# autonomousvision/LaRa

Hardware: AMD Instinct MI355X
Metric: novel-view frames/sec @512x512 (4-view in, 2DGS fwd+bwd) (higher is better)
Workload: dtype f32 raster + bf16-MFMA/f32-accumulate encoder (+ bf16-autocast coarse decoder MLP, as the reference's bf16-mixed)

## Files before the change

include/lara_finedec.h:

```cpp
#ifndef LARA_FINEDEC_H
#define LARA_FINEDEC_H

#include <stdint.h>

#ifdef __cplusplus
extern "C" {
#endif

int lara_fine_decoder_forward(int32_t n, const float *xn, const float *pf, const float *Wqk, const float *W1ov,
                              const float *b1, const float *W2, const float *b2, float *sh, void *stream);

int lara_fine_decoder_backward(int32_t n, const float *xn, const float *pf, const float *Wqk, const float *W1ov,
                               const float *b1, const float *W2, const float *b2, const float *d_sh, float *d_xn,
                               float *d_pf, float *U, float *HID, float *DH, float *DT, void *stream);

int32_t lara_fine_wgrad_floats(void);
int64_t lara_fine_wgrad_workspace_bytes(int32_t n);
int lara_fine_decoder_wgrad(int32_t n, const float *xn, const float *U, const float *HID, const float *DH, const float *DT,
                            const float *d_sh, float *out, void *workspace, void *stream);

int32_t lara_fine_ln_blocks(int32_t n);
int lara_fine_ln_forward(int32_t n, const float *x, const float *gamma, const float *beta, float eps, float *xn,
                         float *stats, void *stream);
int lara_fine_ln_backward(int32_t n, const float *x, const float *gamma, const float *stats, const float *d_xn,
                          float *d_x, float *partials, void *stream);

#ifdef __cplusplus
}
#endif
#endif
```

lara_amd/csrc/finedec.hip:

```cpp
#include "common.h"
#include "../../include/lara_finedec.h"

namespace {

constexpr int FD = 80, NH = 8, CD = 8, NV = 4, HID = 64, SH = 12, TQ = NH * CD;

typedef float f32x16 __attribute__((ext_vector_type(16)));

__device__ __forceinline__ int crow(const int tile, const int r, const int hf) { return tile * 32 + (r >> 2) * 8 + hf * 4 + (r & 3); }
__device__ __forceinline__ f32x16 mfma2(const float a, const float b, const f32x16 c) {
    return __builtin_amdgcn_mfma_f32_32x32x2f32(a, b, c, 0, 0, 0);
}
#define FD_FENCE(i, every) do { if (((i) % (every)) == (every) - 1) asm volatile("" ::: "memory"); } while (0)

__device__ __forceinline__ f32x16 zero16() {
    f32x16 z;
#pragma unroll
    for (int i = 0; i < 16; i++) z[i] = 0.f;
    return z;
}

constexpr int L_WQKT = 0;
constexpr int L_W1T = L_WQKT + FD * TQ;
constexpr int L_W2T = L_W1T + TQ * HID;
// ... 26 lines not shown
    for (int k = 0; k < 10; k++) { const float4 v = x4[k]; xh[4 * k] = v.x; xh[4 * k + 1] = v.y; xh[4 * k + 2] = v.z; xh[4 * k + 3] = v.w; }
}

__device__ __forceinline__ void folded_queries(const float *sw, const float xh[40], const int col, const int hf, f32x16 t[2]) {
    t[0] = zero16(); t[1] = zero16();
#pragma unroll
    for (int s = 0; s < 40; s++) {
        const float *w = sw + L_WQKT + (hf * 40 + s) * TQ + col;
        t[0] = mfma2(w[0], xh[s], t[0]);
        t[1] = mfma2(w[32], xh[s], t[1]);
        FD_FENCE(s, 4);
    }
}

__device__ __forceinline__ void load_pf_half(const float *pf_g, const int64_t n, const int64_t pt, const int hf, float pf[NV][4]) {
#pragma unroll
    for (int j = 0; j < NV; j++)
#pragma unroll
        for (int c = 0; c < 4; c++) pf[j][c] = pf_g[(int64_t)(j * CD + hf * 4 + c) * n + pt];
}

__device__ __forceinline__ float other_half(const float x) { return __shfl_xor(x, 32, 64); }

__device__ __forceinline__ void attention_weights(const f32x16 t[2], const float pf[NV][4], float p[NH][NV]) {
#pragma unroll
    for (int h = 0; h < NH; h++) {
        float sc[NV], m = -1e30f;
#pragma unroll
        for (int j = 0; j < NV; j++) {
            float a = 0.f;
#pragma unroll
            for (int c = 0; c < 4; c++) a += t[h >> 2][(h & 3) * 4 + c] * pf[j][c];
            a += other_half(a);
            sc[j] = a;
            m = fmaxf(m, a);
        }
        float z = 0.f;
#pragma unroll
        for (int j = 0; j < NV; j++) { p[h][j] = __expf(sc[j] - m); z += p[h][j]; }
        const float rz = 1.0f / z;
#pragma unroll
        for (int j = 0; j < NV; j++) p[h][j] *= rz;
    }
}

__device__ __forceinline__ void attend(const float p[NH][NV], const float pf[NV][4], f32x16 u[2]) {
#pragma unroll
    for (int h = 0; h < NH; h++)
#pragma unroll
        for (int c = 0; c < 4; c++)
            u[h >> 2][(h & 3) * 4 + c] = p[h][0] * pf[0][c] + p[h][1] * pf[1][c] + p[h][2] * pf[2][c] + p[h][3] * pf[3][c];
}

__device__ __forceinline__ void hidden_pre(const float *sw, const f32x16 u[2], const int col, const int hf, f32x16 hid[2]) {
    hid[0] = zero16(); hid[1] = zero16();
#pragma unroll
    for (int mt = 0; mt < 2; mt++)
#pragma unroll
        for (int r = 0; r < 16; r++) {
            const float *w = sw + L_W1T + crow(mt, r, hf) * HID + col;
            hid[0] = mfma2(w[0], u[mt][r], hid[0]);
            hid[1] = mfma2(w[32], u[mt][r], hid[1]);
            FD_FENCE(r, 4);
        }
#pragma unroll
    for (int mt = 0; mt < 2; mt++)
#pragma unroll
        for (int r = 0; r < 16; r++) hid[mt][r] += sw[L_B1 + crow(mt, r, hf)];
}

__global__ void __launch_bounds__(256) __attribute__((amdgpu_waves_per_eu(2, 2)))
fine_decoder_fwd_kernel(const int n, const float *__restrict__ xn_g, const float *__restrict__ pf_g,
                        const float *__restrict__ Wqk, const float *__restrict__ W1ov, const float *__restrict__ b1,
                        const float *__restrict__ W2, const float *__restrict__ b2, float *__restrict__ sh_g) {
    __shared__ __attribute__((aligned(16))) float sw[L_FWD_END];
    stage_weights(sw, Wqk, W1ov, b1, W2, b2, false);
    const int lane = threadIdx.x & 63, col = lane & 31, hf = lane >> 5, wave = threadIdx.x >> 6;
    for (int64_t base = (int64_t)blockIdx.x * 128; base < n; base += (int64_t)gridDim.x * 128) {
        const int64_t pt = base + wave * 32 + col;
        const bool live = pt < n;
        const int64_t ptc = live ? pt : (int64_t)n - 1;
        float xh[40];
        load_xn_half(xn_g, ptc, hf, xh);
        f32x16 tu[2];
        folded_queries(sw, xh, col, hf, tu);
        {
            float pf[NV][4], p[NH][NV];
            load_pf_half(pf_g, n, ptc, hf, pf);
            attention_weights(tu, pf, p);
            attend(p, pf, tu);
        }
        f32x16 hid[2];
        hidden_pre(sw, tu, col, hf, hid);
        f32x16 out = zero16();
#pragma unroll
        for (int mt = 0; mt < 2; mt++)
#pragma unroll
            for (int r = 0; r < 16; r++) {
                out = mfma2(sw[L_W2T + crow(mt, r, hf) * 32 + col], fmaxf(hid[mt][r], 0.f), out);
                FD_FENCE(r, 8);
            }
        if (live) {
            float4 *o4 = (float4 *)(sh_g + pt * SH);
            const float *bb = sw + L_B2;
            o4[hf] = make_float4(out[0] + bb[4 * hf], out[1] + bb[4 * hf + 1], out[2] + bb[4 * hf + 2], out[3] + bb[4 * hf + 3]);
            if (hf == 0) o4[2] = make_float4(out[4] + bb[8], out[5] + bb[9], out[6] + bb[10], out[7] + bb[11]);
        }
    }
}

__global__ void __launch_bounds__(256)
fine_decoder_bwd_kernel(const int n, const float *__restrict__ xn_g, const float *__restrict__ pf_g,
                        const float *__restrict__ Wqk, const float *__restrict__ W1ov, const float *__restrict__ b1,
                        const float *__restrict__ W2, const float *__restrict__ b2, const float *__restrict__ dsh_g,
                        float *__restrict__ dxn_g, float *__restrict__ dpf_g, float *__restrict__ U_g,
                        float *__restrict__ H_g, float *__restrict__ DH_g, float *__restrict__ DT_g) {
    extern __shared__ __attribute__((aligned(16))) float sw[];
    stage_weights(sw, Wqk, W1ov, b1, W2, b2, true);
    const int lane = threadIdx.x & 63, col = lane & 31, hf = lane >> 5, wave = threadIdx.x >> 6;
    auto store64 = [&](float *g, const int64_t pt, const f32x16 v[2]) {
#pragma unroll
        for (int mt = 0; mt < 2; mt++)
#pragma unroll
            for (int q = 0; q < 4; q++)
                *(float4 *)(g + pt * 64 + mt * 32 + q * 8 + hf * 4) = make_float4(v[mt][4 * q], v[mt][4 * q + 1], v[mt][4 * q + 2], v[mt][4 * q + 3]);
    };
    for (int64_t base = (int64_t)blockIdx.x * 128; base < n; base += (int64_t)gridDim.x * 128) {
        const int64_t pt = base + wave * 32 + col;
        const bool live = pt < n;
        const int64_t ptc = live ? pt : (int64_t)n - 1;
        f32x16 t[2], u[2];
        {
            float xh[40];
            load_xn_half(xn_g, ptc, hf, xh);
            folded_queries(sw, xh, col, hf, t);
        }
        float pf[NV][4], p[NH][NV];
        load_pf_half(pf_g, n, ptc, hf, pf);
        attention_weights(t, pf, p);
        attend(p, pf, u);
        if (live) store64(U_g, pt, u);
        asm volatile("" ::: "memory");
        f32x16 hid[2], dh[2];
        hidden_pre(sw, u, col, hf, hid);
        {
            float ds[8];
            const float4 *d4 = (const float4 *)(dsh_g + ptc * SH);
            if (hf == 0) {
                const float4 a = d4[0], b = d4[1];
                ds[0] = a.x; ds[1] = a.y; ds[2] = a.z; ds[3] = a.w; ds[4] = b.x; ds[5] = b.y; ds[6] = b.z; ds[7] = b.w;
            } else {
                const float4 c = d4[2];
                ds[0] = c.x; ds[1] = c.y; ds[2] = c.z; ds[3] = c.w; ds[4] = ds[5] = ds[6] = ds[7] = 0.f;
            }
            dh[0] = zero16(); dh[1] = zero16();
#pragma unroll
            for (int s_ = 0; s_ < 8; s_++) {
                const float *w = sw + L_W2P + (hf * 8 + s_) * HID + col;
                dh[0] = mfma2(w[0], ds[s_], dh[0]);
                dh[1] = mfma2(w[32], ds[s_], dh[1]);
                FD_FENCE(s_, 4);
// ... 229 lines not shown
            }
        }
        const int kh = lane >> 5;
#pragma unroll
        for (int ea = 0; ea < 2; ea++)
#pragma unroll
            for (int eb = 0; eb < 2; eb++)
#pragma unroll
                for (int e = 0; e < 16; e++) {
                    const int i = 2 * ((e & 3) + 8 * (e >> 2) + 4 * kh) + ea, j = 4 * c + 2 * wave + eb;
                    if (j < FD) out[(size_t)i * FD + j] = acc[ea][eb][e];
                }
    } else {
        f32x16 acc1[2][2], acc2[1][2];
#pragma unroll
        for (int b = 0; b < 2; b++)
#pragma unroll
            for (int e = 0; e < 16; e++) { acc1[0][b][e] = 0.f; acc1[1][b][e] = 0.f; acc2[0][b][e] = 0.f; }
        float cs1x = 0.f, cs1y = 0.f, cs2 = 0.f;
        const bool s_ok = c < SH;
        for (int r = 0; r < rows; r += 2 * UN) {
            float2 dh[UN], uu[UN], hh[UN];
            float ds[UN];
#pragma unroll
            for (int u = 0; u < UN; u++) {
                const int rr = r + 2 * u + kk;
                const bool in = rr < rows;
                const size_t row = (size_t)(row0 + rr);
                dh[u] = in ? *(const float2 *)(DH + row * HID + 2 * c) : make_float2(0.f, 0.f);
                uu[u] = in ? *(const float2 *)(U + row * 64 + 2 * c) : make_float2(0.f, 0.f);
                hh[u] = in ? *(const float2 *)(HID_ + row * HID + 2 * c) : make_float2(0.f, 0.f);
                ds[u] = (in && s_ok) ? d_sh[row * SH + c] : 0.f;
            }
#pragma unroll
            for (int u = 0; u < UN; u++) {
                cs1x += dh[u].x; cs1y += dh[u].y; cs2 += ds[u];
                acc1[0][0] = mfma2(dh[u].x, uu[u].x, acc1[0][0]);
                acc1[0][1] = mfma2(dh[u].x, uu[u].y, acc1[0][1]);
                acc1[1][0] = mfma2(dh[u].y, uu[u].x, acc1[1][0]);
                acc1[1][1] = mfma2(dh[u].y, uu[u].y, acc1[1][1]);
                acc2[0][0] = mfma2(ds[u], hh[u].x, acc2[0][0]);
                acc2[0][1] = mfma2(ds[u], hh[u].y, acc2[0][1]);
            }
        }
        fw_store<2, 2>(out + FW_O_W1, 64, 64, 64, lane, acc1);
        fw_store<1, 2>(out + FW_O_W2, HID, SH, HID, lane, acc2);
        cs1x += __shfl_xor(cs1x, 32, 64); cs1y += __shfl_xor(cs1y, 32, 64); cs2 += __shfl_xor(cs2, 32, 64);
        if (lane < 32) { out[FW_O_B1 + 2 * c] = cs1x; out[FW_O_B1 + 2 * c + 1] = cs1y; }
        if (lane < SH) out[FW_O_B2 + lane] = cs2;
    }
}

__global__ void __launch_bounds__(256)
fine_wgrad_reduce_kernel(const float *__restrict__ part, const int slabs, float *__restrict__ out) {
    __shared__ float ph[4][64];
    const int k = blockIdx.x * 64 + (threadIdx.x & 63), q = threadIdx.x >> 6;
    float a0 = 0.f, a1 = 0.f;
    if (k < FW_OUT) {
        int s = q;
        for (; s + 4 < slabs; s += 8) {
            a0 += part[(size_t)s * FW_OUT + k];
            a1 += part[(size_t)(s + 4) * FW_OUT + k];
        }
        if (s < slabs) a0 += part[(size_t)s * FW_OUT + k];
    }
    ph[q][threadIdx.x & 63] = a0 + a1;
    __syncthreads();
    if (q == 0 && k < FW_OUT) out[k] = (ph[0][threadIdx.x] + ph[1][threadIdx.x]) + (ph[2][threadIdx.x] + ph[3][threadIdx.x]);
}

unsigned fd_grid(int n) {
    const unsigned tiles = (unsigned)((n + 127) / 128);
    return tiles < 1024u ? tiles : 1024u;
}

}

extern "C" {

int lara_fine_decoder_forward(int32_t n, const float *xn, const float *pf, const float *Wqk, const float *W1ov,
                              const float *b1, const float *W2, const float *b2, float *sh, void *stream) {
    if (n < 0) return LARA2DGS_E_INVALID;
    if (n == 0) return LARA2DGS_OK;
    if (!xn || !pf || !Wqk || !W1ov || !b1 || !W2 || !b2 || !sh) return LARA2DGS_E_INVALID;
    hipStream_t s = (hipStream_t)stream;
    {
        L2D_PROF("fine_decoder_fwd", s);
        hipLaunchKernelGGL(fine_decoder_fwd_kernel, dim3(fd_grid(n)), dim3(256), 0, s, n, xn, pf, Wqk, W1ov, b1, W2, b2, sh);
    }
    L2D_CHECK_LAUNCH();
    return LARA2DGS_OK;
}

int lara_fine_decoder_backward(int32_t n, const float *xn, const float *pf, const float *Wqk, const float *W1ov,
                               const float *b1, const float *W2, const float *b2, const float *d_sh, float *d_xn,
                               float *d_pf, float *U, float *HID_, float *DH, float *DT, void *stream) {
    if (n < 0) return LARA2DGS_E_INVALID;
    if (n == 0) return LARA2DGS_OK;
    if (!xn || !pf || !Wqk || !W1ov || !b1 || !W2 || !b2 || !d_sh || !d_xn || !d_pf || !U || !HID_ || !DH || !DT)
        return LARA2DGS_E_INVALID;
    hipStream_t s = (hipStream_t)stream;
    {
        L2D_PROF("fine_decoder_bwd", s);
        static bool lds_set = false;
        if (!lds_set) {
            if (hipFuncSetAttribute((const void *)fine_decoder_bwd_kernel, hipFuncAttributeMaxDynamicSharedMemorySize,
                                    L_BWD_END * 4) != hipSuccess) return LARA2DGS_E_LAUNCH;
            lds_set = true;
        }
        hipLaunchKernelGGL(fine_decoder_bwd_kernel, dim3(fd_grid(n) < 512u ? fd_grid(n) : 512u), dim3(256), L_BWD_END * 4, s, n, xn, pf,
                           Wqk, W1ov, b1, W2, b2, d_sh, d_xn, d_pf, U, HID_, DH, DT);
    }
    L2D_CHECK_LAUNCH();
    return LARA2DGS_OK;
}

int32_t lara_fine_wgrad_floats(void) { return FW_OUT; }
int64_t lara_fine_wgrad_workspace_bytes(int32_t n) { return n <= 0 ? 0 : (int64_t)((n + FW_SLAB - 1) / FW_SLAB) * FW_OUT * 4; }

int lara_fine_decoder_wgrad(int32_t n, const float *xn, const float *U, const float *HID_, const float *DH, const float *DT,
                            const float *d_sh, float *out, void *workspace, void *stream) {
    if (n < 0 || !out) return LARA2DGS_E_INVALID;
    hipStream_t s = (hipStream_t)stream;
    if (n == 0) {
        hipError_t e = hipMemsetAsync(out, 0, (size_t)FW_OUT * 4, s);
        if (e != hipSuccess) { l2d_set_hip_error(e); return LARA2DGS_E_LAUNCH; }
        return LARA2DGS_OK;
    }
    if (!xn || !U || !HID_ || !DH || !DT || !d_sh || !workspace) return LARA2DGS_E_INVALID;
    const int slabs = (n + FW_SLAB - 1) / FW_SLAB;
    {
        L2D_PROF("fine_decoder_wgrad", s);
        hipLaunchKernelGGL(fine_wgrad_kernel, dim3((unsigned)slabs), dim3(192), 0, s, n, xn, U, HID_, DH, DT, d_sh, (float *)workspace);
        hipLaunchKernelGGL(fine_wgrad_reduce_kernel, dim3((FW_OUT + 63) / 64), dim3(256), 0, s, (const float *)workspace, slabs, out);
    }
    L2D_CHECK_LAUNCH();
    return LARA2DGS_OK;
}

int32_t lara_fine_ln_blocks(int32_t n) { return n <= 0 ? 0 : (n + 255) / 256; }

int lara_fine_ln_forward(int32_t n, const float *x, const float *gamma, const float *beta, float eps, float *xn,
                         float *stats, void *stream) {
    if (n < 0) return LARA2DGS_E_INVALID;
    if (n == 0) return LARA2DGS_OK;
    if (!x || !gamma || !beta || !xn || !stats) return LARA2DGS_E_INVALID;
    hipStream_t s = (hipStream_t)stream;
    {
        L2D_PROF("fine_ln_fwd", s);
        hipLaunchKernelGGL(fine_ln_fwd_kernel, dim3((unsigned)lara_fine_ln_blocks(n)), dim3(256), 0, s, n, x, gamma, beta, eps, xn,
                           (float2 *)stats);
    }
    L2D_CHECK_LAUNCH();
    return LARA2DGS_OK;
}

int lara_fine_ln_backward(int32_t n, const float *x, const float *gamma, const float *stats, const float *d_xn,
                          float *d_x, float *partials, void *stream) {
    if (n < 0) return LARA2DGS_E_INVALID;
    if (n == 0) return LARA2DGS_OK;
    if (!x || !gamma || !stats || !d_xn || !d_x || !partials) return LARA2DGS_E_INVALID;
    hipStream_t s = (hipStream_t)stream;
    {
        L2D_PROF("fine_ln_bwd", s);
        hipLaunchKernelGGL(fine_ln_bwd_kernel, dim3((unsigned)lara_fine_ln_blocks(n)), dim3(256), 0, s, n, x, gamma,
                           (const float2 *)stats, d_xn, d_x, partials);
    }
    L2D_CHECK_LAUNCH();
    return LARA2DGS_OK;
}

}
```

lara_amd/fine.py:

```python
from __future__ import annotations

import ctypes
import math
import os

import torch

from .rasterizer import _check, load_library

_configured = False


def _lib():
    global _configured
    lib = load_library()
    if not _configured:
        vp, i32 = ctypes.c_void_p, ctypes.c_int32
        lib.lara_point_feats_forward.restype = ctypes.c_int
        lib.lara_point_feats_forward.argtypes = [i32, i32, i32, i32] + [vp] * 10
        lib.lara_point_feats_backward.restype = ctypes.c_int
        lib.lara_point_feats_backward.argtypes = [i32, i32, i32, i32] + [vp] * 14
        lib.lara_point_feats_forward_concat.restype = ctypes.c_int
        lib.lara_point_feats_forward_concat.argtypes = [i32, i32, i32, i32, i32] + [vp] * 10
        lib.lara_point_feats_backward_concat.restype = ctypes.c_int
        lib.lara_point_feats_backward_concat.argtypes = [i32, i32, i32, i32, i32] + [vp] * 14
        lib.lara_point_feats_workspace_bytes.restype = ctypes.c_int64
        lib.lara_point_feats_workspace_bytes.argtypes = [i32, i32, i32]
        lib.lara_fine_decoder_forward.restype = ctypes.c_int
        lib.lara_fine_decoder_forward.argtypes = [i32] + [vp] * 9
        lib.lara_fine_decoder_backward.restype = ctypes.c_int
        lib.lara_fine_decoder_backward.argtypes = [i32] + [vp] * 15
        lib.lara_fine_wgrad_floats.restype = i32
        lib.lara_fine_wgrad_workspace_bytes.restype = ctypes.c_int64
        lib.lara_fine_wgrad_workspace_bytes.argtypes = [i32]
        lib.lara_fine_decoder_wgrad.restype = ctypes.c_int
        lib.lara_fine_decoder_wgrad.argtypes = [i32] + [vp] * 9
        lib.lara_fine_ln_blocks.restype = i32
        lib.lara_fine_ln_blocks.argtypes = [i32]
        lib.lara_fine_ln_forward.restype = ctypes.c_int
        lib.lara_fine_ln_forward.argtypes = [i32, vp, vp, vp, ctypes.c_float, vp, vp, vp]
        lib.lara_fine_ln_backward.restype = ctypes.c_int
        lib.lara_fine_ln_backward.argtypes = [i32] + [vp] * 7
        lib.lara_take_rows.restype = ctypes.c_int
        lib.lara_take_rows.argtypes = [i32, vp, i32, ctypes.POINTER(_RowsItem), i32, vp]
        lib.lara_voxel_rows.restype = ctypes.c_int
        lib.lara_voxel_rows.argtypes = [i32, i32, vp, vp, vp, i32, vp]
        _configured = True
    return lib


def _workspace(device, V, h, w):
    n = _lib().lara_point_feats_workspace_bytes(V, h, w)
    if n < 0:
        _check(int(n), "lara_point_feats_workspace_bytes")
    return torch.empty(int(n), dtype=torch.uint8, device=device)


class _PointFeats(torch.autograd.Function):
    @staticmethod
    def forward(ctx, points, w2cs, ixts, img_ref, image, acc_map, depth, row_views):
        if not points.is_cuda:
            raise RuntimeError("lara_amd: tensors must live on an MI355X (HIP) device; there is no CPU path")
        f = lambda t: t.detach().float().contiguous()
        points, w2cs, ixts, img_ref, image, acc_map, depth = map(f, (points, w2cs, ixts, img_ref, image, acc_map, depth))
        n, V, h, w = points.shape[0], img_ref.shape[0], img_ref.shape[2], img_ref.shape[3]
        if points.shape != (n, 3) or w2cs.shape != (V, 4, 4) or ixts.shape != (V, 3, 3) or img_ref.shape != (V, 3, h, w):
            raise RuntimeError("expected points [n,3], w2cs [V,4,4], ixts [V,3,3], img_ref [V,3,h,w]")
        if row_views:
            R = int(row_views)
            if R < V or image.shape != (h, R * w, 3) or acc_map.numel() != h * R * w or depth.shape != (h, R * w, 1):
                raise RuntimeError("expected points [n,3], ... and image [h,R*w,3], acc_map [h,R*w], depth [h,R*w,1] with R = row_views >= V")
        elif image.shape != (V, h, w, 3) or acc_map.shape != (V, h, w) or depth.shape != (V, h, w, 1):
            raise RuntimeError("expected points [n,3], w2cs [V,4,4], ixts [V,3,3], img_ref [V,3,h,w], image [V,h,w,3], acc_map [V,h,w], depth [V,h,w,1]")
        out = torch.empty(V, 8, n, dtype=torch.float32, device=points.device)
        ws = _workspace(points.device, V, h, w)
        with torch.cuda.device(points.device):
            _check(_lib().lara_point_feats_forward_concat(n, V, int(row_views or 0), h, w, points.data_ptr(), w2cs.data_ptr(),
                                                          ixts.data_ptr(), img_ref.data_ptr(), image.data_ptr(), acc_map.data_ptr(),
                                                          depth.data_ptr(), out.data_ptr(), ws.data_ptr(),
                                                          torch.cuda.current_stream(points.device).cuda_stream),
                   "lara_point_feats_forward")
        ctx.save_for_backward(points, w2cs, ixts, img_ref, image, acc_map, depth)
        ctx.row_views = int(row_views or 0)
        return out

    @staticmethod
    def backward(ctx, g_out):
        points, w2cs, ixts, img_ref, image, acc_map, depth = ctx.saved_tensors
        n, V, h, w = points.shape[0], img_ref.shape[0], img_ref.shape[2], img_ref.shape[3]
        g_out = g_out.float().contiguous()
        need = ctx.needs_input_grad
        d_points = torch.empty_like(points)
        maps = [(image, need[4]), (acc_map, need[5]), (depth, need[6])]
        sizes = [(t.numel() + 3) // 4 * 4 if nd else 0 for t, nd in maps]
        flat = torch.zeros(sum(sizes), dtype=torch.float32, device=points.device)
# ... 200 lines not shown
                k *= d
            out.append(dw[o:o + k].view(shape))
            o += k
        return (d_xn, d_pf, *out)


def _tn_over_points(a, b, chunk=1024):
    n = a.shape[0]
    m = n // chunk * chunk
    out = None
    if m:
        out = torch.bmm(a[:m].view(-1, chunk, a.shape[1]).transpose(1, 2), b[:m].view(-1, chunk, b.shape[1])).float().sum(0)
    if m < n:
        tail = (a[m:].t() @ b[m:]).float()
        out = tail if out is None else out + tail
    return out


class _FineLayerNorm(torch.autograd.Function):

    @staticmethod
    def forward(ctx, x, gamma, beta, eps):
        if not x.is_cuda:
            raise RuntimeError("lara_amd: tensors must live on an MI355X (HIP) device; there is no CPU path")
        x, gamma, beta = x.detach().float().contiguous(), gamma.detach().float().contiguous(), beta.detach().float().contiguous()
        n = x.shape[0]
        xn = torch.empty_like(x)
        stats = torch.empty(n, 2, dtype=torch.float32, device=x.device)
        with torch.cuda.device(x.device):
            _check(_lib().lara_fine_ln_forward(n, x.data_ptr(), gamma.data_ptr(), beta.data_ptr(), float(eps), xn.data_ptr(),
                                               stats.data_ptr(), torch.cuda.current_stream(x.device).cuda_stream),
                   "lara_fine_ln_forward")
        ctx.save_for_backward(x, gamma, stats)
        return xn

    @staticmethod
    def backward(ctx, d_xn):
        x, gamma, stats = ctx.saved_tensors
        n = x.shape[0]
        d_xn = d_xn.float().contiguous()
        d_x = torch.empty_like(x)
        lib = _lib()
        parts = torch.empty(max(lib.lara_fine_ln_blocks(n), 1), 2 * _FD, dtype=torch.float32, device=x.device)
        if n == 0:
            parts.zero_()
        with torch.cuda.device(x.device):
            _check(lib.lara_fine_ln_backward(n, x.data_ptr(), gamma.data_ptr(), stats.data_ptr(), d_xn.data_ptr(), d_x.data_ptr(),
                                             parts.data_ptr(), torch.cuda.current_stream(x.device).cuda_stream),
                   "lara_fine_ln_backward")
        tot = parts.sum(0)
        return d_x, tot[:_FD], tot[_FD:], None


def _fold_fine_weights(decoder):
    att = decoder.cross_att
    E = att.embed_dim
    if (E != _FD or att.num_heads != _NH or att.kdim != _CD or att.vdim != _CD or att.in_proj_bias is not None
            or att.out_proj.bias is not None or decoder.mlp_fine[0].out_features != _HID
            or decoder.mlp_fine[2].out_features != _SH):
        raise RuntimeError("lara_amd.fine.forward_fine is built for LaRa's sizes only: embed 80, 8 heads, kdim = vdim = 8, "
                           "no biases in the attention, hidden 64, 12 SH outputs (sh_degree 1)")
    Wq = att.q_proj_weight.float().view(_NH, _HD, E)
    Wk = att.k_proj_weight.float().view(_NH, _HD, _CD)
    Wv = att.v_proj_weight.float().view(_NH, _HD, _CD)
    Wo = att.out_proj.weight.float().view(E, _NH, _HD)
    Wqk = torch.einsum("hdc,hdi->hci", Wk, Wq).reshape(_NH * _CD, E) * (_HD ** -0.5)
    Wov = torch.einsum("ohd,hdc->ohc", Wo, Wv).reshape(E, _NH * _CD)
    W1, b1 = decoder.mlp_fine[0].weight.float(), decoder.mlp_fine[0].bias.float()
    W2, b2 = decoder.mlp_fine[2].weight.float(), decoder.mlp_fine[2].bias.float()
    return Wqk, W1 @ Wov, b1, W2, b2


def fold_fine_weights(decoder):
    return _fold_fine_weights(decoder)


def forward_fine(decoder, volume_feat, point_feats, folded=None):
    if point_feats.dim() != 3 or point_feats.shape[1:] != (_NV, _CD) or volume_feat.shape[-1] != _FD:
        raise RuntimeError("expected volume_feat [n,80] and point_feats [n,4,8]")
    xn = _FineLayerNorm.apply(volume_feat.float(), decoder.norm.weight, decoder.norm.bias, decoder.norm.eps)
    pf = point_feats.float().permute(1, 2, 0)
    sh = _FineDecoder.apply(xn, pf, *(_fold_fine_weights(decoder) if folded is None else folded))
    return sh.unsqueeze(1)
```

Measured before the change: 924.8.

## Fuse fine-decoder LayerNorm with decoder forward and backward into single-stage kernels

Adds a fused fine stage in which the forward kernel computes LayerNorm statistics and normalisation in-register before the folded attention/MLP, storing only per-point mean/rstd instead of a normalised activation tensor. A new backward kernel recomputes the forward, runs the backward through attention, MLP and LayerNorm, and accumulates weight gradients (including gamma/beta) in per-block partials reduced by one kernel. This replaces separate LN forward/backward, decoder backward and wgrad launches, along with their intermediate U/H/DH/DT buffers, cutting launches and global memory traffic. The cost is recompute in the backward, a large LDS footprint that may limit occupancy, and a grid capped at 256 blocks.

After: 909.5. 0.983x the previous value.

```diff
diff --git a/include/lara_finedec.h b/include/lara_finedec.h
--- a/include/lara_finedec.h
+++ b/include/lara_finedec.h
@@ -25,6 +25,15 @@
 int lara_fine_ln_backward(int32_t n, const float *x, const float *gamma, const float *stats, const float *d_xn,
                           float *d_x, float *partials, void *stream);
 
+int32_t lara_fine_stage_grid(int32_t n);
+int64_t lara_fine_stage_workspace_bytes(int32_t n);
+int lara_fine_stage_forward(int32_t n, const float *x, const float *gamma, const float *beta, float eps, const float *pf,
+                            const float *Wqk, const float *W1ov, const float *b1, const float *W2, const float *b2, float *sh,
+                            float *stats, void *stream);
+int lara_fine_stage_backward(int32_t n, const float *x, const float *gamma, const float *beta, const float *stats, const float *pf,
+                             const float *Wqk, const float *W1ov, const float *b1, const float *W2, const float *b2,
+                             const float *d_sh, float *d_x, float *d_pf, float *out, void *workspace, void *stream);
+
 #ifdef __cplusplus
 }
 #endif
diff --git a/lara_amd/csrc/finedec.hip b/lara_amd/csrc/finedec.hip
--- a/lara_amd/csrc/finedec.hip
+++ b/lara_amd/csrc/finedec.hip
@@ -102,7 +102,8 @@
             u[h >> 2][(h & 3) * 4 + c] = p[h][0] * pf[0][c] + p[h][1] * pf[1][c] + p[h][2] * pf[2][c] + p[h][3] * pf[3][c];
 }
 
-__device__ __forceinline__ void hidden_pre(const float *sw, const f32x16 u[2], const int col, const int hf, f32x16 hid[2]) {
+__device__ __forceinline__ void hidden_pre(const float *sw, const f32x16 u[2], const int col, const int hf, f32x16 hid[2],
+                                           const int lb1 = L_B1) {
     hid[0] = zero16(); hid[1] = zero16();
 #pragma unroll
     for (int mt = 0; mt < 2; mt++)
@@ -116,22 +117,49 @@
 #pragma unroll
     for (int mt = 0; mt < 2; mt++)
 #pragma unroll
-        for (int r = 0; r < 16; r++) hid[mt][r] += sw[L_B1 + crow(mt, r, hf)];
-}
-
-__global__ void __launch_bounds__(256) __attribute__((amdgpu_waves_per_eu(2, 2)))
-fine_decoder_fwd_kernel(const int n, const float *__restrict__ xn_g, const float *__restrict__ pf_g,
-                        const float *__restrict__ Wqk, const float *__restrict__ W1ov, const float *__restrict__ b1,
-                        const float *__restrict__ W2, const float *__restrict__ b2, float *__restrict__ sh_g) {
-    __shared__ __attribute__((aligned(16))) float sw[L_FWD_END];
-    stage_weights(sw, Wqk, W1ov, b1, W2, b2, false);
+        for (int r = 0; r < 16; r++) hid[mt][r] += sw[lb1 + crow(mt, r, hf)];
+}
+
+__device__ __forceinline__ void row_stats(const float xh[40], const float eps, float &mean, float &rstd) {
+    float sum = 0.f;
+#pragma unroll
+    for (int k = 0; k < 10; k++) sum += (xh[4 * k] + xh[4 * k + 1]) + (xh[4 * k + 2] + xh[4 * k + 3]);
+    sum += other_half(sum);
+    mean = sum * (1.0f / FD);
+    asm volatile("" : "+v"(mean));
+    float var = 0.f;
+#pragma unroll
+    for (int k = 0; k < 10; k++) {
+        const float a = xh[4 * k] - mean, b = xh[4 * k + 1] - mean, c = xh[4 * k + 2] - mean, d = xh[4 * k + 3] - mean;
+        var += (a * a + b * b) + (c * c + d * d);
+    }
+    var += other_half(var);
+    rstd = 1.0f / sqrtf(var * (1.0f / FD) + eps);
+}
+
+__device__ __forceinline__ void normalise_half(float xh[40], const float mean, const float rstd, const float *g, const float *b,
+                                               const int hf) {
+#pragma unroll
+    for (int s = 0; s < 40; s++) xh[s] = (xh[s] - mean) * rstd * g[hf * 40 + s] + b[hf * 40 + s];
+}
+
+template <bool LN>
+__device__ __forceinline__ void decoder_fwd_tiles(const float *sw, const float *sgb, const int n, const float *__restrict__ x_g,
+                                                  const float eps, float2 *__restrict__ stats, const float *__restrict__ pf_g,
+                                                  float *__restrict__ sh_g) {
     const int lane = threadIdx.x & 63, col = lane & 31, hf = lane >> 5, wave = threadIdx.x >> 6;
     for (int64_t base = (int64_t)blockIdx.x * 128; base < n; base += (int64_t)gridDim.x * 128) {
         const int64_t pt = base + wave * 32 + col;
         const bool live = pt < n;
         const int64_t ptc = live ? pt : (int64_t)n - 1;
         float xh[40];
-        load_xn_half(xn_g, ptc, hf, xh);
+        load_xn_half(x_g, ptc, hf, xh);
+        if (LN) {
+            float mean, rstd;
+            row_stats(xh, eps, mean, rstd);
+            normalise_half(xh, mean, rstd, sgb, sgb + FD, hf);
+            if (live && hf == 0) stats[pt] = make_float2(mean, rstd);
+        }
         f32x16 tu[2];
         folded_queries(sw, xh, col, hf, tu);
         {
@@ -157,6 +185,27 @@
             if (hf == 0) o4[2] = make_float4(out[4] + bb[8], out[5] + bb[9], out[6] + bb[10], out[7] + bb[11]);
         }
     }
+}
+
+__global__ void __launch_bounds__(256) __attribute__((amdgpu_waves_per_eu(2, 2)))
+fine_decoder_fwd_kernel(const int n, const float *__restrict__ xn_g, const float *__restrict__ pf_g,
+                        const float *__restrict__ Wqk, const float *__restrict__ W1ov, const float *__restrict__ b1,
+                        const float *__restrict__ W2, const float *__restrict__ b2, float *__restrict__ sh_g) {
+    __shared__ __attribute__((aligned(16))) float sw[L_FWD_END];
+    stage_weights(sw, Wqk, W1ov, b1, W2, b2, false);
+    decoder_fwd_tiles<false>(sw, nullptr, n, xn_g, 0.f, nullptr, pf_g, sh_g);
+}
+
+__global__ void __launch_bounds__(256) __attribute__((amdgpu_waves_per_eu(2, 2)))
+fine_stage_fwd_kernel(const int n, const float *__restrict__ x_g, const float *__restrict__ gamma, const float *__restrict__ beta,
+                      const float eps, const float *__restrict__ pf_g, const float *__restrict__ Wqk,
+                      const float *__restrict__ W1ov, const float *__restrict__ b1, const float *__restrict__ W2,
+                      const float *__restrict__ b2, float *__restrict__ sh_g, float2 *__restrict__ stats) {
+    __shared__ __attribute__((aligned(16))) float sw[L_FWD_END];
+    __shared__ float sgb[2 * FD];
+    if (threadIdx.x < FD) { sgb[threadIdx.x] = gamma[threadIdx.x]; sgb[FD + threadIdx.x] = beta[threadIdx.x]; }
+    stage_weights(sw, Wqk, W1ov, b1, W2, b2, false);
+    decoder_fwd_tiles<true>(sw, sgb, n, x_g, eps, stats, pf_g, sh_g);
 }
 
 __global__ void __launch_bounds__(256)
@@ -492,21 +541,344 @@
 }
 
 __global__ void __launch_bounds__(256)
-fine_wgrad_reduce_kernel(const float *__restrict__ part, const int slabs, float *__restrict__ out) {
+fine_wgrad_reduce_kernel(const float *__restrict__ part, const int slabs, const int width, float *__restrict__ out) {
     __shared__ float ph[4][64];
     const int k = blockIdx.x * 64 + (threadIdx.x & 63), q = threadIdx.x >> 6;
     float a0 = 0.f, a1 = 0.f;
-    if (k < FW_OUT) {
+    if (k < width) {
         int s = q;
         for (; s + 4 < slabs; s += 8) {
-            a0 += part[(size_t)s * FW_OUT + k];
-            a1 += part[(size_t)(s + 4) * FW_OUT + k];
-        }
-        if (s < slabs) a0 += part[(size_t)s * FW_OUT + k];
+            a0 += part[(size_t)s * width + k];
+            a1 += part[(size_t)(s + 4) * width + k];
+        }
+        if (s < slabs) a0 += part[(size_t)s * width + k];
     }
     ph[q][threadIdx.x & 63] = a0 + a1;
     __syncthreads();
-    if (q == 0 && k < FW_OUT) out[k] = (ph[0][threadIdx.x] + ph[1][threadIdx.x]) + (ph[2][threadIdx.x] + ph[3][threadIdx.x]);
+    if (q == 0 && k < width) out[k] = (ph[0][threadIdx.x] + ph[1][threadIdx.x]) + (ph[2][threadIdx.x] + ph[3][threadIdx.x]);
+}
+
+constexpr int FS_OUT = FW_OUT + 2 * FD;
+constexpr unsigned FS_MAX_GRID = 256;
+constexpr int Q_B1 = L_W1T + TQ * HID;
+constexpr int Q_W2P = Q_B1 + HID;
+constexpr int Q_W1 = Q_W2P + 16 * HID;
+constexpr int Q_WQK = Q_W1 + HID * TQ;
+constexpr int Q_G = Q_WQK + TQ * 96;
+constexpr int Q_GB = Q_G + 2 * FD;
+constexpr int Q_STAGE = Q_GB + 4 * 2 * FD;
+constexpr int S_LD = 68, S_LDX = 84, S_LDS = 20;
+constexpr int S_B = 32 * S_LD;
+constexpr int S_WAVE = S_B + 32 * S_LDX;
+constexpr int Q_END = Q_STAGE + 4 * S_WAVE;
+static_assert(Q_END * 4 <= 160 * 1024, "LDS");
+static_assert(Q_STAGE % 4 == 0 && S_WAVE % 4 == 0 && S_B % 4 == 0, "float4 stores into the stage");
+static_assert(12 * 1024 + HID + 16 <= 4 * S_WAVE, "the cross-wave sum reuses the stages");
+
+__device__ __forceinline__ void wave_lds_handover() { asm volatile("s_waitcnt lgkmcnt(0)" ::: "memory"); }
+
+template <int NA, int NB>
+__device__ __forceinline__ void contract_points(const float *A, const int lda, const int a_cols, const float *B, const int ldb,
+                                                const int b_cols, const int col, const int hf, f32x16 (&acc)[NA][NB],
+                                                float (&cs)[NA]) {
+#pragma unroll
+    for (int s = 0; s < 16; s++) {
+        const int row = 2 * s + hf;
+        float a[NA], b[NB];
+#pragma unroll
+        for (int ia = 0; ia < NA; ia++) {
+            a[ia] = 32 * ia + col < a_cols ? A[row * lda + 32 * ia + col] : 0.f;
+            cs[ia] += a[ia];
+        }
+#pragma unroll
+        for (int jb = 0; jb < NB; jb++) b[jb] = 32 * jb + col < b_cols ? B[row * ldb + 32 * jb + col] : 0.f;
+#pragma unroll
+        for (int ia = 0; ia < NA; ia++)
+#pragma unroll
+            for (int jb = 0; jb < NB; jb++) acc[ia][jb] = mfma2(a[ia], b[jb], acc[ia][jb]);
+        FD_FENCE(s, 1);
+    }
+}
+
+__device__ __forceinline__ float half_wave_sum(float x) {
+    x += dpp_term<0xB1, 0xf>(x);
+    x += dpp_term<0x4E, 0xf>(x);
+    x += dpp_term<0x141, 0xf>(x);
+    x += dpp_term<0x140, 0xf>(x);
+    x += dpp_term<0x142, 0xa>(x);
+    return x;
+}
+
+__global__ void __launch_bounds__(256)
+fine_stage_bwd_kernel(const int n, const float *__restrict__ x_g, const float *__restrict__ gamma, const float *__restrict__ beta,
+                      const float2 *__restrict__ stats, const float *__restrict__ pf_g, const float *__restrict__ Wqk,
+                      const float *__restrict__ W1ov, const float *__restrict__ b1, const float *__restrict__ W2,
+                      const float *__restrict__ dsh_g, float *__restrict__ dx_g, float *__restrict__ dpf_g,
+                      float *__restrict__ part) {
+    extern __shared__ __attribute__((aligned(16))) float sw[];
+    for (int i = threadIdx.x; i < TQ * FD; i += blockDim.x) sw[L_WQKT + (i % FD) * TQ + i / FD] = Wqk[i];
+    for (int i = threadIdx.x; i < HID * TQ; i += blockDim.x) { sw[L_W1T + (i % TQ) * HID + i / TQ] = W1ov[i]; sw[Q_W1 + i] = W1ov[i]; }
+    for (int i = threadIdx.x; i < HID; i += blockDim.x) sw[Q_B1 + i] = b1[i];
+    for (int i = threadIdx.x; i < 16 * HID; i += blockDim.x) sw[Q_W2P + i] = i < SH * HID ? W2[i] : 0.f;
+    for (int i = threadIdx.x; i < TQ * 96; i += blockDim.x) sw[Q_WQK + i] = (i % 96) < FD ? Wqk[(i / 96) * FD + i % 96] : 0.f;
+    for (int i = threadIdx.x; i < FD; i += blockDim.x) { sw[Q_G + i] = gamma[i]; sw[Q_G + FD + i] = beta[i]; }
+    for (int i = threadIdx.x; i < 4 * 2 * FD; i += blockDim.x) sw[Q_GB + i] = 0.f;
+    __syncthreads();
+    const int lane = threadIdx.x & 63, wave = threadIdx.x >> 6;
+    int col = lane & 31, hf = lane >> 5;
+    const float *sg = sw + Q_G, *sb = sw + Q_G + FD;
+    float *gb = sw + Q_GB + wave * 2 * FD;
+    float *st = sw + Q_STAGE + wave * S_WAVE;
+    auto stage64 = [&](float *dst, const f32x16 v[2], const bool keep) {
+#pragma unroll
+        for (int mt = 0; mt < 2; mt++)
+#pragma unroll
+            for (int q = 0; q < 4; q++)
+                *(float4 *)(dst + col * S_LD + mt * 32 + q * 8 + hf * 4) =
+                    keep ? make_float4(v[mt][4 * q], v[mt][4 * q + 1], v[mt][4 * q + 2], v[mt][4 * q + 3]) : make_float4(0.f, 0.f, 0.f, 0.f);
+    };
+    f32x16 aqk[2][3], aw1[2][2], aw2[1][2];
+#pragma unroll
+    for (int a = 0; a < 2; a++) {
+#pragma unroll
+        for (int b = 0; b < 3; b++) aqk[a][b] = zero16();
+#pragma unroll
+        for (int b = 0; b < 2; b++) aw1[a][b] = zero16();
+    }
+    aw2[0][0] = zero16(); aw2[0][1] = zero16();
+    float cb1[2] = {0.f, 0.f}, cb2[1] = {0.f};
+
+    for (int64_t base = (int64_t)blockIdx.x * 128; base < n; base += (int64_t)gridDim.x * 128) {
+        asm volatile("" : "+v"(col), "+v"(hf));
+        const int64_t pt = base + wave * 32 + col;
+        const bool live = pt < n;
+        const int64_t ptc = live ? pt : (int64_t)n - 1;
+        const float2 ms = stats[ptc];
+        f32x16 t[2], u[2];
+        {
+            float xh[40];
+            load_xn_half(x_g, ptc, hf, xh);
+            normalise_half(xh, ms.x, ms.y, sg, sb, hf);
+            folded_queries(sw, xh, col, hf, t);
+        }
+        float pf[NV][4], p[NH][NV];
+        load_pf_half(pf_g, n, ptc, hf, pf);
+        attention_weights(t, pf, p);
+        attend(p, pf, u);
+        wave_lds_handover();
+        stage64(st + S_B, u, true);
+        f32x16 hid[2], dh[2];
+        hidden_pre(sw, u, col, hf, hid, Q_B1);
+        float ds[8];
+        {
+            const float4 *d4 = (const float4 *)(dsh_g + ptc * SH);
+            if (hf == 0) {
+                const float4 a = d4[0], b = d4[1];
+                ds[0] = a.x; ds[1] = a.y; ds[2] = a.z; ds[3] = a.w; ds[4] = b.x; ds[5] = b.y; ds[6] = b.z; ds[7] = b.w;
+            } else {
+                const float4 c = d4[2];
+                ds[0] = c.x; ds[1] = c.y; ds[2] = c.z; ds[3] = c.w; ds[4] = ds[5] = ds[6] = ds[7] = 0.f;
+            }
+            dh[0] = zero16(); dh[1] = zero16();
+#pragma unroll
+            for (int s_ = 0; s_ < 8; s_++) {
+                const float *w = sw + Q_W2P + (hf * 8 + s_) * HID + col;
+                dh[0] = mfma2(w[0], ds[s_], dh[0]);
+                dh[1] = mfma2(w[32], ds[s_], dh[1]);
+                FD_FENCE(s_, 4);
+            }
+        }
+#pragma unroll
+        for (int mt = 0; mt < 2; mt++)
+#pragma unroll
+            for (int r = 0; r < 16; r++) {
+                const bool on = hid[mt][r] > 0.f;
+                hid[mt][r] = on ? hid[mt][r] : 0.f;
+                dh[mt][r] = on ? dh[mt][r] : 0.f;
+            }
+        stage64(st, dh, live);
+        wave_lds_handover();
+        contract_points<2, 2>(st, S_LD, HID, st + S_B, S_LD, TQ, col, hf, aw1, cb1);
+        wave_lds_handover();
+        stage64(st + S_B, hid, true);
+        {
+            float *d = st + col * S_LDS + hf * 8;
+            *(float4 *)d = live ? make_float4(ds[0], ds[1], ds[2], ds[3]) : make_float4(0.f, 0.f, 0.f, 0.f);
+            if (hf == 0) *(float4 *)(d + 4) = live ? make_float4(ds[4], ds[5], ds[6], ds[7]) : make_float4(0.f, 0.f, 0.f, 0.f);
+        }
+        wave_lds_handover();
+        contract_points<1, 2>(st, S_LDS, SH, st + S_B, S_LD, HID, col, hf, aw2, cb2);
+        f32x16 du[2];
+        du[0] = zero16(); du[1] = zero16();
+#pragma unroll
+        for (int mt = 0; mt < 2; mt++)
+#pragma unroll
+            for (int r = 0; r < 16; r++) {
+                const float *w = sw + Q_W1 + crow(mt, r, hf) * TQ + col;
+                du[0] = mfma2(w[0], dh[mt][r], du[0]);
+                du[1] = mfma2(w[32], dh[mt][r], du[1]);
+                FD_FENCE(r, 4);
+            }
+        asm volatile("" ::: "memory");
+        float dpf[NV][4];
+#pragma unroll
+        for (int j = 0; j < NV; j++)
+#pragma unroll
+            for (int c = 0; c < 4; c++) dpf[j][c] = 0.f;
+#pragma unroll
+        for (int h = 0; h < NH; h++) {
+            const int mt = h >> 2, r0 = (h & 3) * 4;
+            float dp[NV], dot = 0.f;
+#pragma unroll
+            for (int j = 0; j < NV; j++) {
+                float a = 0.f;
+#pragma unroll
+                for (int c = 0; c < 4; c++) a += du[mt][r0 + c] * pf[j][c];
+                a += other_half(a);
+                dp[j] = a;
+                dot += p[h][j] * a;
+            }
+            float dt[4] = {0.f, 0.f, 0.f, 0.f};
+#pragma unroll
+            for (int j = 0; j < NV; j++) {
+                const float dsc = p[h][j] * (dp[j] - dot);
+#pragma unroll
+                for (int c = 0; c < 4; c++) {
+                    dt[c] += dsc * pf[j][c];
+                    dpf[j][c] += p[h][j] * du[mt][r0 + c] + dsc * t[mt][r0 + c];
+                }
+            }
+#pragma unroll
+            for (int c = 0; c < 4; c++) du[mt][r0 + c] = dt[c];
+            asm volatile("" ::: "memory");
+        }
+        if (live) {
+#pragma unroll
+            for (int j = 0; j < NV; j++)
+#pragma unroll
+                for (int c = 0; c < 4; c++) dpf_g[(int64_t)(j * CD + hf * 4 + c) * n + pt] = dpf[j][c];
+        }
+        f32x16 xa[3];
+        wave_lds_handover();
+#pragma unroll
+        for (int ft = 0; ft < 3; ft++)
+#pragma unroll
+            for (int q = 0; q < 4; q++)
+                if (ft * 32 + q * 8 < FD) {
+                    const int f0 = ft * 32 + q * 8 + hf * 4;
+                    const float4 v = *(const float4 *)(x_g + ptc * FD + f0);
+                    const float xv[4] = {v.x, v.y, v.z, v.w};
+                    float xn[4];
+#pragma unroll
+                    for (int c = 0; c < 4; c++) {
+                        xa[ft][4 * q + c] = (xv[c] - ms.x) * ms.y;
+                        xn[c] = (xv[c] - ms.x) * ms.y * sg[f0 + c] + sb[f0 + c];
+                    }
+                    *(float4 *)(st + S_B + col * S_LDX + f0) = make_float4(xn[0], xn[1], xn[2], xn[3]);
+                }
+        stage64(st, du, live);
+        wave_lds_handover();
+        {
+            float unused[2] = {0.f, 0.f};
+            contract_points<2, 3>(st, S_LD, TQ, st + S_B, S_LDX, FD, col, hf, aqk, unused);
+        }
+        f32x16 dxn[3];
+#pragma unroll
+        for (int ft = 0; ft < 3; ft++) {
+            dxn[ft] = zero16();
+#pragma unroll
+            for (int mt = 0; mt < 2; mt++)
+#pragma unroll
+                for (int r = 0; r < 16; r++) {
+                    dxn[ft] = mfma2(sw[Q_WQK + crow(mt, r, hf) * 96 + ft * 32 + col], du[mt][r], dxn[ft]);
+                    FD_FENCE(r, 8);
+                }
+        }
+        float s1 = 0.f, s2 = 0.f;
+#pragma unroll
+        for (int ft = 0; ft < 3; ft++)
+#pragma unroll
+            for (int q = 0; q < 4; q++)
+                if (ft * 32 + q * 8 < FD) {
+                    const int f0 = ft * 32 + q * 8 + hf * 4;
+                    float g[4];
+#pragma unroll
+                    for (int c = 0; c < 4; c++) {
+                        const int r = 4 * q + c;
+                        const float dv = live ? dxn[ft][r] : 0.f;
+                        const float a = half_wave_sum(dv * xa[ft][r]), b = half_wave_sum(dv);
+                        if (col == 31) { gb[f0 + c] += a; gb[FD + f0 + c] += b; }
+                        g[c] = dv * sg[f0 + c];
+                        dxn[ft][r] = g[c];
+                    }
+                    s1 += (g[0] + g[1]) + (g[2] + g[3]);
+                    s2 += (g[0] * xa[ft][4 * q] + g[1] * xa[ft][4 * q + 1]) + (g[2] * xa[ft][4 * q + 2] + g[3] * xa[ft][4 * q + 3]);
+                }
+        s1 += other_half(s1);
+        s2 += other_half(s2);
+        if (live) {
+            const float m1 = s1 * (1.0f / FD), m2 = s2 * (1.0f / FD);
+#pragma unroll
+            for (int ft = 0; ft < 3; ft++)
+#pragma unroll
+                for (int q = 0; q < 4; q++)
+                    if (ft * 32 + q * 8 < FD) {
+                        const int f0 = ft * 32 + q * 8 + hf * 4, r = 4 * q;
+                        *(float4 *)(dx_g + pt * FD + f0) =
+                            make_float4(ms.y * (dxn[ft][r] - m1 - xa[ft][r] * m2), ms.y * (dxn[ft][r + 1] - m1 - xa[ft][r + 1] * m2),
+                                        ms.y * (dxn[ft][r + 2] - m1 - xa[ft][r + 2] * m2), ms.y * (dxn[ft][r + 3] - m1 - xa[ft][r + 3] * m2));
+                    }
+        }
+    }
+
+    float *buf = sw + Q_STAGE, *cbuf = buf + 12 * 1024;
+    cb1[0] += other_half(cb1[0]); cb1[1] += other_half(cb1[1]); cb2[0] += other_half(cb2[0]);
+    for (int w = 0; w < 4; w++) {
+        __syncthreads();
+        if (wave == w) {
+            auto add = [&](const int tile, const f32x16 &v) {
+#pragma unroll
+                for (int r = 0; r < 16; r++) {
+                    float *d = buf + (tile * 16 + r) * 64 + lane;
+                    *d = w ? *d + v[r] : v[r];
+                }
+            };
+#pragma unroll
+            for (int a = 0; a < 2; a++) {
+#pragma unroll
+                for (int b = 0; b < 3; b++) add(a * 3 + b, aqk[a][b]);
+#pragma unroll
+                for (int b = 0; b < 2; b++) add(6 + a * 2 + b, aw1[a][b]);
+            }
+            add(10, aw2[0][0]); add(11, aw2[0][1]);
+            if (hf == 0) {
+                cbuf[col] = w ? cbuf[col] + cb1[0] : cb1[0];
+                cbuf[32 + col] = w ? cbuf[32 + col] + cb1[1] : cb1[1];
+                if (col < SH) cbuf[HID + col] = w ? cbuf[HID + col] + cb2[0] : cb2[0];
+            }
+        }
+    }
+    __syncthreads();
+    float *out = part + (size_t)blockIdx.x * FS_OUT;
+    for (int e = threadIdx.x; e < 12 * 1024; e += blockDim.x) {
+        const int tile = e >> 10, r = (e >> 6) & 15, l = e & 63;
+        const int i = 8 * (r >> 2) + 4 * (l >> 5) + (r & 3), j = l & 31;
+        const float v = buf[e];
+        if (tile < 6) {
+            const int q = 32 * (tile / 3) + i, f = 32 * (tile % 3) + j;
+            if (f < FD) out[q * FD + f] = v;
+        } else if (tile < 10) {
+            out[FW_O_W1 + (32 * ((tile - 6) >> 1) + i) * TQ + 32 * ((tile - 6) & 1) + j] = v;
+        } else if (i < SH) {
+            out[FW_O_W2 + i * HID + 32 * (tile - 10) + j] = v;
+        }
+    }
+    if (threadIdx.x < HID) out[FW_O_B1 + threadIdx.x] = cbuf[threadIdx.x];
+    if (threadIdx.x < SH) out[FW_O_B2 + threadIdx.x] = cbuf[HID + threadIdx.x];
+    if (threadIdx.x < 2 * FD) {
+        const float *g4 = sw + Q_GB + threadIdx.x;
+        out[FW_OUT + threadIdx.x] = ((g4[0] + g4[2 * FD]) + g4[4 * FD]) + g4[6 * FD];
+    }
 }
 
 unsigned fd_grid(int n) {
@@ -572,7 +944,7 @@
     {
         L2D_PROF("fine_decoder_wgrad", s);
         hipLaunchKernelGGL(fine_wgrad_kernel, dim3((unsigned)slabs), dim3(192), 0, s, n, xn, U, HID_, DH, DT, d_sh, (float *)workspace);
-        hipLaunchKernelGGL(fine_wgrad_reduce_kernel, dim3((FW_OUT + 63) / 64), dim3(256), 0, s, (const float *)workspace, slabs, out);
+        hipLaunchKernelGGL(fine_wgrad_reduce_kernel, dim3((FW_OUT + 63) / 64), dim3(256), 0, s, (const float *)workspace, slabs, FW_OUT, out);
     }
     L2D_CHECK_LAUNCH();
     return LARA2DGS_OK;
@@ -610,4 +982,56 @@
     return LARA2DGS_OK;
 }
 
-}
+int32_t lara_fine_stage_grid(int32_t n) {
+    if (n <= 0) return 0;
+    const unsigned g = fd_grid(n);
+    return (int32_t)(g < FS_MAX_GRID ? g : FS_MAX_GRID);
+}
+int64_t lara_fine_stage_workspace_bytes(int32_t n) { return (int64_t)lara_fine_stage_grid(n) * FS_OUT * 4; }
+
+int lara_fine_stage_forward(int32_t n, const float *x, const float *gamma, const float *beta, float eps, const float *pf,
+                            const float *Wqk, const float *W1ov, const float *b1, const float *W2, const float *b2, float *sh,
+                            float *stats, void *stream) {
+    if (n < 0) return LARA2DGS_E_INVALID;
+    if (n == 0) return LARA2DGS_OK;
+    if (!x || !gamma || !beta || !pf || !Wqk || !W1ov || !b1 || !W2 || !b2 || !sh || !stats) return LARA2DGS_E_INVALID;
+    hipStream_t s = (hipStream_t)stream;
+    {
+        L2D_PROF("fine_stage_fwd", s);
+        hipLaunchKernelGGL(fine_stage_fwd_kernel, dim3(fd_grid(n)), dim3(256), 0, s, n, x, gamma, beta, eps, pf, Wqk, W1ov, b1, W2, b2,
+                           sh, (float2 *)stats);
+    }
+    L2D_CHECK_LAUNCH();
+    return LARA2DGS_OK;
+}
+
+int lara_fine_stage_backward(int32_t n, const float *x, const float *gamma, const float *beta, const float *stats, const float *pf,
+                             const float *Wqk, const float *W1ov, const float *b1, const float *W2, const float *b2,
+                             const float *d_sh, float *d_x, float *d_pf, float *out, void *workspace, void *stream) {
+    if (n < 0 || !out) return LARA2DGS_E_INVALID;
+    hipStream_t s = (hipStream_t)stream;
+    if (n == 0) {
+        hipError_t e = hipMemsetAsync(out, 0, (size_t)FS_OUT * 4, s);
+        if (e != hipSuccess) { l2d_set_hip_error(e); return LARA2DGS_E_LAUNCH; }
+        return LARA2DGS_OK;
+    }
+    if (!x || !gamma || !beta || !stats || !pf || !Wqk || !W1ov || !b1 || !W2 || !b2 || !d_sh || !d_x || !d_pf || !workspace)
+        return LARA2DGS_E_INVALID;
+    const int grid = lara_fine_stage_grid(n);
+    {
+        L2D_PROF("fine_stage_bwd", s);
+        static bool lds_set = false;
+        if (!lds_set) {
+            if (hipFuncSetAttribute((const void *)fine_stage_bwd_kernel, hipFuncAttributeMaxDynamicSharedMemorySize, Q_END * 4) !=
+                hipSuccess) return LARA2DGS_E_LAUNCH;
+            lds_set = true;
+        }
+        hipLaunchKernelGGL(fine_stage_bwd_kernel, dim3((unsigned)grid), dim3(256), Q_END * 4, s, n, x, gamma, beta,
+                           (const float2 *)stats, pf, Wqk, W1ov, b1, W2, d_sh, d_x, d_pf, (float *)workspace);
+        hipLaunchKernelGGL(fine_wgrad_reduce_kernel, dim3((FS_OUT + 63) / 64), dim3(256), 0, s, (const float *)workspace, grid, FS_OUT, out);
+    }
+    L2D_CHECK_LAUNCH();
+    return LARA2DGS_OK;
+}
+
+}
diff --git a/lara_amd/fine.py b/lara_amd/fine.py
--- a/lara_amd/fine.py
+++ b/lara_amd/fine.py
@@ -41,6 +41,14 @@
         lib.lara_fine_ln_forward.argtypes = [i32, vp, vp, vp, ctypes.c_float, vp, vp, vp]
         lib.lara_fine_ln_backward.restype = ctypes.c_int
         lib.lara_fine_ln_backward.argtypes = [i32] + [vp] * 7
+        lib.lara_fine_stage_grid.restype = i32
+        lib.lara_fine_stage_grid.argtypes = [i32]
+        lib.lara_fine_stage_workspace_bytes.restype = ctypes.c_int64
+        lib.lara_fine_stage_workspace_bytes.argtypes = [i32]
+        lib.lara_fine_stage_forward.restype = ctypes.c_int
+        lib.lara_fine_stage_forward.argtypes = [i32, vp, vp, vp, ctypes.c_float] + [vp] * 9
+        lib.lara_fine_stage_backward.restype = ctypes.c_int
+        lib.lara_fine_stage_backward.argtypes = [i32] + [vp] * 16
         lib.lara_take_rows.restype = ctypes.c_int
         lib.lara_take_rows.argtypes = [i32, vp, i32, ctypes.POINTER(_RowsItem), i32, vp]
         lib.lara_voxel_rows.restype = ctypes.c_int
@@ -347,6 +355,72 @@
         return d_x, tot[:_FD], tot[_FD:], None
 
 
+fused_fine_stage = True
+
+_scratch = {}
+
+
+def _stage_workspace(dev, stream, nbytes):
+    key = (dev.index, stream)
+    t = _scratch.get(key)
+    if t is None or t.numel() < nbytes:
+        t = torch.empty(max(int(nbytes), 16), dtype=torch.uint8, device=dev)
+        _scratch[key] = t
+    return t
+
+
+def _f32c(t):
+    t = t.detach()
+    return t if t.dtype == torch.float32 and t.is_contiguous() else t.float().contiguous()
+
+
+class _FineStage(torch.autograd.Function):
+
+    @staticmethod
+    def forward(ctx, x, gamma, beta, eps, pf, Wqk, W1ov, b1, W2, b2):
+        if not x.is_cuda:
+            raise RuntimeError("lara_amd: tensors must live on an MI355X (HIP) device; there is no CPU path")
+        x, gamma, beta, pf, Wqk, W1ov, b1, W2, b2 = map(_f32c, (x, gamma, beta, pf, Wqk, W1ov, b1, W2, b2))
+        n = x.shape[0]
+        if (x.shape != (n, _FD) or gamma.shape != (_FD,) or beta.shape != (_FD,) or pf.shape != (_NV, _CD, n)
+                or Wqk.shape != (_NH * _CD, _FD) or W1ov.shape != (_HID, _NH * _CD) or b1.shape != (_HID,)
+                or W2.shape != (_SH, _HID) or b2.shape != (_SH,)):
+            raise RuntimeError("lara_fine_stage_forward: the kernel is built for x [n,80], gamma / beta [80], pf [4,8,n], "
+                               "Wqk [64,80], W1ov [64,64], b1 [64], W2 [12,64], b2 [12]")
+        sh = torch.empty(n, _SH, dtype=torch.float32, device=x.device)
+        stats = torch.empty(n, 2, dtype=torch.float32, device=x.device)
+        if n:
+            with torch.cuda.device(x.device):
+                _check(_lib().lara_fine_stage_forward(n, x.data_ptr(), gamma.data_ptr(), beta.data_ptr(), float(eps), pf.data_ptr(),
+                                                      Wqk.data_ptr(), W1ov.data_ptr(), b1.data_ptr(), W2.data_ptr(), b2.data_ptr(),
+                                                      sh.data_ptr(), stats.data_ptr(),
+                                                      torch.cuda.current_stream(x.device).cuda_stream), "lara_fine_stage_forward")
+        ctx.save_for_backward(x, gamma, beta, stats, pf, Wqk, W1ov, b1, W2, b2)
+        return sh
+
+    @staticmethod
+    def backward(ctx, d_sh):
+        x, gamma, beta, stats, pf, Wqk, W1ov, b1, W2, b2 = ctx.saved_tensors
+        n, dev = x.shape[0], x.device
+        d_sh = _f32c(d_sh)
+        lib = _lib()
+        d_x, d_pf = torch.empty_like(x), torch.empty_like(pf)
+        dw = torch.empty(lib.lara_fine_wgrad_floats() + 2 * _FD, dtype=torch.float32, device=dev)
+        with torch.cuda.device(dev):
+            stream = torch.cuda.current_stream(dev).cuda_stream
+            ws = _stage_workspace(dev, stream, lib.lara_fine_stage_workspace_bytes(n))
+            _check(lib.lara_fine_stage_backward(n, x.data_ptr(), gamma.data_ptr(), beta.data_ptr(), stats.data_ptr(), pf.data_ptr(),
+                                                Wqk.data_ptr(), W1ov.data_ptr(), b1.data_ptr(), W2.data_ptr(), b2.data_ptr(),
+                                                d_sh.data_ptr(), d_x.data_ptr(), d_pf.data_ptr(), dw.data_ptr(), ws.data_ptr(),
+                                                stream), "lara_fine_stage_backward")
+        out, o = [], 0
+        for shape in ((_NH * _CD, _FD), (_HID, _NH * _CD), (_HID,), (_SH, _HID), (_SH,), (_FD,), (_FD,)):
+            k = math.prod(shape)
+            out.append(dw[o:o + k].view(shape))
+            o += k
+        return (d_x, out[5], out[6], None, d_pf, *out[:5])
+
+
 def _fold_fine_weights(decoder):
     att = decoder.cross_att
     E = att.embed_dim
@@ -373,7 +447,11 @@
 def forward_fine(decoder, volume_feat, point_feats, folded=None):
     if point_feats.dim() != 3 or point_feats.shape[1:] != (_NV, _CD) or volume_feat.shape[-1] != _FD:
         raise RuntimeError("expected volume_feat [n,80] and point_feats [n,4,8]")
-    xn = _FineLayerNorm.apply(volume_feat.float(), decoder.norm.weight, decoder.norm.bias, decoder.norm.eps)
     pf = point_feats.float().permute(1, 2, 0)
-    sh = _FineDecoder.apply(xn, pf, *(_fold_fine_weights(decoder) if folded is None else folded))
+    folded = _fold_fine_weights(decoder) if folded is None else folded
+    if fused_fine_stage:
+        sh = _FineStage.apply(volume_feat.float(), decoder.norm.weight, decoder.norm.bias, decoder.norm.eps, pf, *folded)
+    else:
+        xn = _FineLayerNorm.apply(volume_feat.float(), decoder.norm.weight, decoder.norm.bias, decoder.norm.eps)
+        sh = _FineDecoder.apply(xn, pf, *folded)
     return sh.unsqueeze(1)
```
